# CFGpp-diffusion/CFGpp

Measured on NVIDIA H100. Metric: images/sec (device-timed) SDXL 1024x1024 NFE=50 ddim_cfg++, higher is better.
Workload: dtype f16

## Files before the change

cfgpp_b200/csrc/attention.cu:

```cuda
#include <cmath>

#include "attention.cuh"
#include "common.cuh"

namespace cfgpp {

void attn_configure();

namespace {

constexpr int BQ = 64;
constexpr int BKV = 64;
constexpr int kThreads = 128;
constexpr int ATOM_BYTES = 64 * 64 * 2;

template <int HD>
struct ACfg {
  static constexpr int NA = HD / 64;
  static constexpr int TILE_BYTES = NA * ATOM_BYTES;
  static constexpr int SMEM_BYTES = TILE_BYTES * 5 + 1024 + 64;
  static_assert(SMEM_BYTES <= 232448, "shared memory overflow");
};

CFGPP_DEVICE uint32_t tile_off(int row, int chunk) {
  return (chunk >> 3) * ATOM_BYTES + row * 128 + (((chunk & 7) ^ (row & 7)) << 4);
}

template <int HD, bool IP>
CFGPP_DEVICE void attn_body(const AttnParams& p, const CUtensorMap* map_q, const CUtensorMap* map_k,
                            const CUtensorMap* map_v, const CUtensorMap* map_k2, const CUtensorMap* map_v2) {
  using A = ACfg<HD>;
  constexpr int NA = A::NA;
  constexpr int TILE_BYTES = A::TILE_BYTES;
  extern __shared__ uint8_t smem_raw[];
  const uint32_t raw_addr = smem_u32(smem_raw);
  uint8_t* smem = smem_raw + (((raw_addr + 1023u) & ~1023u) - raw_addr);
  uint8_t* sQ = smem;
  uint8_t* sK = sQ + TILE_BYTES;
  uint8_t* sV = sK + 2 * TILE_BYTES;
  uint64_t* bars = reinterpret_cast<uint64_t*>(sV + 2 * TILE_BYTES);
  uint64_t* q_full = bars;
  uint64_t* kv_full = bars + 1;

  const int warp = threadIdx.x >> 5;
  const int lane = threadIdx.x & 31;
  const int q0 = blockIdx.x * BQ;
  const int head = blockIdx.y;
  const int batch = blockIdx.z;
  const int n_tiles = (p.Nkv + BKV - 1) / BKV;

  if (threadIdx.x == 0) {
    tma_prefetch_desc(map_q);
    tma_prefetch_desc(map_k);
    tma_prefetch_desc(map_v);
    mbar_init(q_full, 1);
    mbar_init(&kv_full[0], 1);
    mbar_init(&kv_full[1], 1);
    fence_barrier_init();
  }
  __syncthreads();
  pdl_launch_dependents();
  pdl_wait();
  const float ip_scale = IP ? *p.ip_scale : 0.f;
  const bool ip = IP && ip_scale != 0.f;
  const int n_fills = n_tiles + (ip ? 1 : 0);

  auto load_kv = [&](int j) {
    const int s = j & 1;
    const bool image = IP && j == n_tiles;
    const CUtensorMap* mk = image ? map_k2 : map_k;
    const CUtensorMap* mv = image ? map_v2 : map_v;
    const int row = image ? 0 : j * BKV;
    mbar_arrive_expect_tx(&kv_full[s], 2 * TILE_BYTES);
#pragma unroll
    for (int a = 0; a < NA; ++a) {
      tma_load_3d(sK + s * TILE_BYTES + a * ATOM_BYTES, mk, &kv_full[s], head * HD + a * 64, row, batch);
      tma_load_3d(sV + s * TILE_BYTES + a * ATOM_BYTES, mv, &kv_full[s], head * HD + a * 64, row, batch);
    }
  };
  if (threadIdx.x == 0) {
    if (IP) {
      tma_prefetch_desc(map_k2);
      tma_prefetch_desc(map_v2);
    }
    mbar_arrive_expect_tx(q_full, TILE_BYTES);
#pragma unroll
    for (int a = 0; a < NA; ++a) tma_load_3d(sQ + a * ATOM_BYTES, map_q, q_full, head * HD + a * 64, q0, batch);
    load_kv(0);
    if (n_fills > 1) load_kv(1);
  }

  const float c = p.scale_log2e;
  float o[HD / 8][4];
#pragma unroll
  for (int n = 0; n < HD / 8; ++n) o[n][0] = o[n][1] = o[n][2] = o[n][3] = 0.f;
  float m_run[2] = {-INFINITY, -INFINITY}, l_run[2] = {0.f, 0.f};
  const uint32_t q_base = smem_u32(sQ);
  const int qrow_ld = warp * 16 + (lane & 15);
  auto scores = [&](uint32_t k_base, int valid, float (&sc)[BKV / 8][4]) {
#pragma unroll
    for (int n = 0; n < BKV / 8; ++n) sc[n][0] = sc[n][1] = sc[n][2] = sc[n][3] = 0.f;
#pragma unroll
    for (int kk = 0; kk < HD / 16; ++kk) {
      uint32_t a[4];
      ldmatrix_x4(q_base + tile_off(qrow_ld, 2 * kk + (lane >> 4)), a[0], a[1], a[2], a[3]);
#pragma unroll
      for (int n2 = 0; n2 < BKV / 16; ++n2) {
        const int krow = n2 * 16 + (lane & 7) + ((lane >> 4) << 3);
        uint32_t b0, b1, b2, b3;
        ldmatrix_x4(k_base + tile_off(krow, 2 * kk + ((lane >> 3) & 1)), b0, b1, b2, b3);
        mma_16816(sc[2 * n2], a, b0, b1);
        mma_16816(sc[2 * n2 + 1], a, b2, b3);
      }
    }
    if (valid < BKV) {
#pragma unroll
      for (int n = 0; n < BKV / 8; ++n) {
        const int col = n * 8 + 2 * (lane & 3);
        if (col >= valid) sc[n][0] = sc[n][2] = -INFINITY;
        if (col + 1 >= valid) sc[n][1] = sc[n][3] = -INFINITY;
      }
    }
  };
  mbar_wait(q_full, 0);

  for (int j = 0; j < n_tiles; ++j) {
    const int s = j & 1;
    mbar_wait(&kv_full[s], (j >> 1) & 1);
    const uint32_t k_base = smem_u32(sK + s * TILE_BYTES);
    const uint32_t v_base = smem_u32(sV + s * TILE_BYTES);
    float sc[BKV / 8][4];
    scores(k_base, p.Nkv - j * BKV, sc);
    float alpha[2];
#pragma unroll
    for (int h = 0; h < 2; ++h) {
      float mx = -INFINITY;
#pragma unroll
      for (int n = 0; n < BKV / 8; ++n) mx = fmaxf(mx, fmaxf(sc[n][2 * h], sc[n][2 * h + 1]));
      mx = fmaxf(mx, __shfl_xor_sync(0xffffffffu, mx, 1));
      mx = fmaxf(mx, __shfl_xor_sync(0xffffffffu, mx, 2));
      const float m_new = fmaxf(m_run[h], mx);
      alpha[h] = fast_exp2((m_run[h] - m_new) * c);
      m_run[h] = m_new;
    }
    float rs[2] = {0.f, 0.f};
    uint32_t pa[BKV / 8][2];
#pragma unroll
    for (int n = 0; n < BKV / 8; ++n) {
#pragma unroll
      for (int h = 0; h < 2; ++h) {
        const float mc = m_run[h] * c;
        const float p0 = fast_exp2(sc[n][2 * h] * c - mc);
        const float p1 = fast_exp2(sc[n][2 * h + 1] * c - mc);
        rs[h] += p0 + p1;
        pa[n][h] = pack_half2(p0, p1);
      }
    }
#pragma unroll
    for (int h = 0; h < 2; ++h) l_run[h] = l_run[h] * alpha[h] + rs[h];
#pragma unroll
    for (int n = 0; n < HD / 8; ++n) {
      o[n][0] *= alpha[0];
      o[n][1] *= alpha[0];
      o[n][2] *= alpha[1];
      o[n][3] *= alpha[1];
    }
#pragma unroll
    for (int t = 0; t < BKV / 16; ++t) {
      const uint32_t a[4] = {pa[2 * t][0], pa[2 * t][1], pa[2 * t + 1][0], pa[2 * t + 1][1]};
      const int vrow = t * 16 + (lane & 7) + (((lane >> 3) & 1) << 3);
#pragma unroll
      for (int d2 = 0; d2 < HD / 16; ++d2) {
        uint32_t b0, b1, b2, b3;
        ldmatrix_x4_trans(v_base + tile_off(vrow, 2 * d2 + (lane >> 4)), b0, b1, b2, b3);
        mma_16816(o[2 * d2], a, b0, b1);
        mma_16816(o[2 * d2 + 1], a, b2, b3);
      }
    }
    __syncthreads();
    if (threadIdx.x == 0 && j + 2 < n_fills) load_kv(j + 2);
  }

  float inv_l[2];
#pragma unroll
  for (int h = 0; h < 2; ++h) {
    float l = l_run[h];
    l += __shfl_xor_sync(0xffffffffu, l, 1);
    l += __shfl_xor_sync(0xffffffffu, l, 2);
    inv_l[h] = 1.0f / l;
  }
  if (ip) {
    const int s = n_tiles & 1;
    mbar_wait(&kv_full[s], (n_tiles >> 1) & 1);
    const uint32_t v_base = smem_u32(sV + s * TILE_BYTES);
    float sc[BKV / 8][4];
    scores(smem_u32(sK + s * TILE_BYTES), p.Nkv2, sc);
    float mc[2], inv_l2[2];
#pragma unroll
    for (int h = 0; h < 2; ++h) {
      float mx = -INFINITY;
#pragma unroll
      for (int n = 0; n < BKV / 8; ++n) mx = fmaxf(mx, fmaxf(sc[n][2 * h], sc[n][2 * h + 1]));
      mx = fmaxf(mx, __shfl_xor_sync(0xffffffffu, mx, 1));
      mx = fmaxf(mx, __shfl_xor_sync(0xffffffffu, mx, 2));
      mc[h] = mx * c;
    }
    float rs[2] = {0.f, 0.f};
    uint32_t pa[BKV / 8][2];
#pragma unroll
    for (int n = 0; n < BKV / 8; ++n) {
#pragma unroll
      for (int h = 0; h < 2; ++h) {
        const float p0 = fast_exp2(sc[n][2 * h] * c - mc[h]);
        const float p1 = fast_exp2(sc[n][2 * h + 1] * c - mc[h]);
        rs[h] += p0 + p1;
        pa[n][h] = pack_half2(p0, p1);
      }
    }
#pragma unroll
    for (int h = 0; h < 2; ++h) {
      float l = rs[h];
      l += __shfl_xor_sync(0xffffffffu, l, 1);
      l += __shfl_xor_sync(0xffffffffu, l, 2);
      inv_l2[h] = 1.0f / l;
    }
    const int k_steps = (p.Nkv2 + 15) / 16;
#pragma unroll
    for (int d2 = 0; d2 < HD / 16; ++d2) {
      float acc[2][4] = {{0.f, 0.f, 0.f, 0.f}, {0.f, 0.f, 0.f, 0.f}};
#pragma unroll
      for (int t = 0; t < BKV / 16; ++t) {
        if (t >= k_steps) break;
        const uint32_t a[4] = {pa[2 * t][0], pa[2 * t][1], pa[2 * t + 1][0], pa[2 * t + 1][1]};
        const int vrow = t * 16 + (lane & 7) + (((lane >> 3) & 1) << 3);
        uint32_t b0, b1, b2, b3;
        ldmatrix_x4_trans(v_base + tile_off(vrow, 2 * d2 + (lane >> 4)), b0, b1, b2, b3);
        mma_16816(acc[0], a, b0, b1);
        mma_16816(acc[1], a, b2, b3);
      }
#pragma unroll
      for (int i = 0; i < 2; ++i)
#pragma unroll
        for (int e = 0; e < 4; ++e)
          o[2 * d2 + i][e] = o[2 * d2 + i][e] * inv_l[e >> 1] + ip_scale * (acc[i][e] * inv_l2[e >> 1]);
    }
    inv_l[0] = inv_l[1] = 1.0f;
  }
#pragma unroll
  for (int h = 0; h < 2; ++h) {
    const int qrow = q0 + warp * 16 + (lane >> 2) + 8 * h;
    if (qrow >= p.Nq) continue;
    __half* dst = p.out + (static_cast<size_t>(batch) * p.Nq + qrow) * p.ldo + head * HD + 2 * (lane & 3);
#pragma unroll
    for (int n = 0; n < HD / 8; ++n)
      *reinterpret_cast<uint32_t*>(dst + n * 8) = pack_half2(o[n][2 * h] * inv_l[h], o[n][2 * h + 1] * inv_l[h]);
  }
}

template <int HD>
__global__ void __launch_bounds__(kThreads)
attn_kernel(const AttnParams p, const __grid_constant__ CUtensorMap map_q, const __grid_constant__ CUtensorMap map_k,
            const __grid_constant__ CUtensorMap map_v) {
  attn_body<HD, false>(p, &map_q, &map_k, &map_v, nullptr, nullptr);
}

template <int HD>
__global__ void __launch_bounds__(kThreads)
attn_ip_kernel(const AttnParams p, const __grid_constant__ CUtensorMap map_q, const __grid_constant__ CUtensorMap map_k,
               const __grid_constant__ CUtensorMap map_v, const __grid_constant__ CUtensorMap map_k2,
               const __grid_constant__ CUtensorMap map_v2) {
  attn_body<HD, true>(p, &map_q, &map_k, &map_v, &map_k2, &map_v2);
}

CUtensorMap make_head_map(const __half* base, int ld, int B, int N, int cols) {
  uint64_t dims[3] = {(uint64_t)cols, (uint64_t)N, (uint64_t)B};
  uint64_t strides[2] = {(uint64_t)ld * 2, (uint64_t)N * ld * 2};
  uint32_t box[3] = {64, 64, 1};
  return make_tmap_f16(base, 3, dims, strides, box);
}

template <int HD>
void configure_one() {
  CFGPP_CHECK_CUDA(cudaFuncSetAttribute(attn_kernel<HD>, cudaFuncAttributeMaxDynamicSharedMemorySize,
                                        ACfg<HD>::SMEM_BYTES));
  CFGPP_CHECK_CUDA(cudaFuncSetAttribute(attn_ip_kernel<HD>, cudaFuncAttributeMaxDynamicSharedMemorySize,
                                        ACfg<HD>::SMEM_BYTES));
}

template <int HD>
void launch(const AttnOp& op, cudaStream_t stream) {
  dim3 grid((op.p.Nq + BQ - 1) / BQ, op.p.H, op.p.B);
  if (op.p.ip_scale)
    launch_pdl(attn_ip_kernel<HD>, grid, dim3(kThreads), ACfg<HD>::SMEM_BYTES, stream, op.p, op.map_q, op.map_k,
               op.map_v, op.map_k2, op.map_v2);
  else
    launch_pdl(attn_kernel<HD>, grid, dim3(kThreads), ACfg<HD>::SMEM_BYTES, stream, op.p, op.map_q, op.map_k,
               op.map_v);
}

}

int attn_padded_head_dim(int head_dim) { return ((head_dim + 63) / 64) * 64; }

AttnOp make_attn_op(const __half* q, int ldq, const __half* k, int ldk, const __half* v, int ldv, __half* out,
                    int ldo, int B, int H, int Nq, int Nkv, int head_dim) {
  AttnOp op{};
  CFGPP_REQUIRE(Nkv >= 1 && Nq >= 1, "empty attention");
  CFGPP_REQUIRE(ldo % 8 == 0, "ldo must be a multiple of 8");
  CFGPP_REQUIRE(head_dim >= 8 && head_dim <= 192, "attention supports head_dim <= 192");
  const int hdp = attn_padded_head_dim(head_dim);
  op.hd_pad = hdp;
  op.head_dim = head_dim;
  op.p.B = B; op.p.H = H; op.p.Nq = Nq; op.p.Nkv = Nkv; op.p.ldo = ldo; op.p.out = out;
  op.p.scale_log2e = (1.0f / sqrtf(static_cast<float>(head_dim))) * 1.4426950408889634f;
  op.map_q = make_head_map(q, ldq, B, Nq, H * hdp);
  op.map_k = make_head_map(k, ldk, B, Nkv, H * hdp);
  op.map_v = make_head_map(v, ldv, B, Nkv, H * hdp);
  return op;
}

AttnOp make_attn_ip_op(const __half* q, int ldq, const __half* k, int ldk, const __half* v, int ldv, const __half* k2,
                       int ldk2, const __half* v2, int ldv2, int Nkv2, const float* ip_scale, __half* out, int ldo,
                       int B, int H, int Nq, int Nkv, int head_dim) {
  CFGPP_REQUIRE(Nkv2 >= 1 && Nkv2 <= 64, "the image segment holds 1..64 tokens");
  CFGPP_REQUIRE(ip_scale != nullptr, "the image segment needs its scale word");
  AttnOp op = make_attn_op(q, ldq, k, ldk, v, ldv, out, ldo, B, H, Nq, Nkv, head_dim);
  op.p.Nkv2 = Nkv2;
  op.p.ip_scale = ip_scale;
  op.map_k2 = make_head_map(k2, ldk2, B, Nkv2, H * op.hd_pad);
  op.map_v2 = make_head_map(v2, ldv2, B, Nkv2, H * op.hd_pad);
  return op;
}

void attn_configure() {
  static bool done = false;
  if (done) return;
  configure_one<64>();
  configure_one<128>();
  configure_one<192>();
  done = true;
}

void run_attn_op(const AttnOp& op, cudaStream_t stream) {
  attn_configure();
  switch (op.hd_pad) {
    case 64: return launch<64>(op, stream);
    case 128: return launch<128>(op, stream);
    case 192: return launch<192>(op, stream);
    default: throw Error(-1, "unsupported padded head dim");
  }
}

}
```

cfgpp_b200/csrc/common.cuh:

```cuda
#pragma once
#include <cuda.h>
#include <cuda_fp16.h>
#include <cuda_runtime.h>
#include <stdint.h>
#include <stdio.h>

namespace cfgpp {

#define CFGPP_DEVICE __device__ __forceinline__

CFGPP_DEVICE uint32_t smem_u32(const void* p) {
  return static_cast<uint32_t>(__cvta_generic_to_shared(p));
}

CFGPP_DEVICE void pdl_launch_dependents() { asm volatile("griddepcontrol.launch_dependents;" ::: "memory"); }
CFGPP_DEVICE void pdl_wait() { asm volatile("griddepcontrol.wait;" ::: "memory"); }

CFGPP_DEVICE void mbar_init(uint64_t* bar, uint32_t count) {
  asm volatile("mbarrier.init.shared::cta.b64 [%0], %1;" ::"r"(smem_u32(bar)), "r"(count));
}
CFGPP_DEVICE void fence_barrier_init() {
  asm volatile("fence.mbarrier_init.release.cluster;" ::: "memory");
}
CFGPP_DEVICE void mbar_arrive_expect_tx(uint64_t* bar, uint32_t bytes) {
  asm volatile("mbarrier.arrive.expect_tx.shared::cta.b64 _, [%0], %1;" ::"r"(smem_u32(bar)), "r"(bytes)
               : "memory");
}
CFGPP_DEVICE void mbar_arrive(uint64_t* bar) {
  asm volatile("mbarrier.arrive.shared::cta.b64 _, [%0];" ::"r"(smem_u32(bar)) : "memory");
}
CFGPP_DEVICE uint32_t mbar_try_wait(uint64_t* bar, uint32_t parity) {
  uint32_t ok;
  asm volatile(
      "{\n\t"
      ".reg .pred P1;\n\t"
      "mbarrier.try_wait.parity.shared::cta.b64 P1, [%1], %2;\n\t"
      "selp.u32 %0, 1, 0, P1;\n\t"
      "}"
      : "=r"(ok)
      : "r"(smem_u32(bar)), "r"(parity)
      : "memory");
  return ok;
}
#ifndef CFGPP_MBAR_SLEEP_NS
#define CFGPP_MBAR_SLEEP_NS 1000000
#endif
CFGPP_DEVICE uint32_t mbar_try_wait_sleep(uint64_t* bar, uint32_t parity) {
  uint32_t ok;
  asm volatile(
      "{\n\t"
      ".reg .pred P1;\n\t"
      "mbarrier.try_wait.parity.shared::cta.b64 P1, [%1], %2, %3;\n\t"
      "selp.u32 %0, 1, 0, P1;\n\t"
      "}"
      : "=r"(ok)
      : "r"(smem_u32(bar)), "r"(parity), "r"(CFGPP_MBAR_SLEEP_NS)
      : "memory");
  return ok;
}
CFGPP_DEVICE void mbar_wait(uint64_t* bar, uint32_t parity) {
  if (mbar_try_wait(bar, parity)) return;
  const long long t0 = clock64();
#if CFGPP_MBAR_SLEEP_NS > 0
  while (!mbar_try_wait_sleep(bar, parity)) {
#else
  while (!mbar_try_wait(bar, parity)) {
#endif
    if (clock64() - t0 > 4000000000LL) {
      printf("cfgpp: mbarrier wait timeout (block %d thread %d bar 0x%x parity %u)\n", blockIdx.x, threadIdx.x,
             smem_u32(bar), parity);
      __trap();
    }
  }
}

CFGPP_DEVICE void mbar_wait_nocall(uint64_t* bar, uint32_t parity) {
  if (mbar_try_wait(bar, parity)) return;
  const long long t0 = clock64();
  while (!mbar_try_wait(bar, parity)) {
    if (clock64() - t0 > 4000000000LL) __trap();
  }
}

CFGPP_DEVICE void tma_prefetch_desc(const CUtensorMap* map) {
  asm volatile("prefetch.tensormap [%0];" ::"l"(reinterpret_cast<uint64_t>(map)) : "memory");
}
CFGPP_DEVICE void tma_load_2d(void* smem_dst, const CUtensorMap* map, uint64_t* bar, int c0, int c1) {
  asm volatile(
      "cp.async.bulk.tensor.2d.shared::cluster.global.mbarrier::complete_tx::bytes [%0], [%1, {%3, %4}], [%2];"
      ::"r"(smem_u32(smem_dst)), "l"(reinterpret_cast<uint64_t>(map)), "r"(smem_u32(bar)), "r"(c0), "r"(c1)
      : "memory");
}
CFGPP_DEVICE void tma_load_3d(void* smem_dst, const CUtensorMap* map, uint64_t* bar, int c0, int c1, int c2) {
  asm volatile(
      "cp.async.bulk.tensor.3d.shared::cluster.global.mbarrier::complete_tx::bytes [%0], [%1, {%3, %4, %5}], [%2];"
      ::"r"(smem_u32(smem_dst)), "l"(reinterpret_cast<uint64_t>(map)), "r"(smem_u32(bar)), "r"(c0), "r"(c1),
      "r"(c2)
      : "memory");
}
CFGPP_DEVICE void tma_load_4d(void* smem_dst, const CUtensorMap* map, uint64_t* bar, int c0, int c1, int c2,
                              int c3) {
  asm volatile(
      "cp.async.bulk.tensor.4d.shared::cluster.global.mbarrier::complete_tx::bytes [%0], [%1, {%3, %4, %5, %6}], "
      "[%2];" ::"r"(smem_u32(smem_dst)),
      "l"(reinterpret_cast<uint64_t>(map)), "r"(smem_u32(bar)), "r"(c0), "r"(c1), "r"(c2), "r"(c3)
      : "memory");
}
CFGPP_DEVICE void tma_load_im2col_4d(void* smem_dst, const CUtensorMap* map, uint64_t* bar, int c, int w, int h, int n,
                                     uint16_t off_w, uint16_t off_h) {
  asm volatile(
      "cp.async.bulk.tensor.4d.shared::cluster.global.im2col.mbarrier::complete_tx::bytes [%0], [%1, {%3, %4, %5, %6}], "
      "[%2], {%7, %8};" ::"r"(smem_u32(smem_dst)),
      "l"(reinterpret_cast<uint64_t>(map)), "r"(smem_u32(bar)), "r"(c), "r"(w), "r"(h), "r"(n), "h"(off_w), "h"(off_h)
      : "memory");
}

CFGPP_DEVICE void tma_store_2d(const CUtensorMap* map, const void* smem_src, int c0, int c1) {
  asm volatile("cp.async.bulk.tensor.2d.global.shared::cta.bulk_group [%0, {%2, %3}], [%1];" ::"l"(
                   reinterpret_cast<uint64_t>(map)),
               "r"(smem_u32(smem_src)), "r"(c0), "r"(c1)
               : "memory");
}
CFGPP_DEVICE void tma_store_commit() { asm volatile("cp.async.bulk.commit_group;" ::: "memory"); }
CFGPP_DEVICE void tma_store_wait_read0() { asm volatile("cp.async.bulk.wait_group.read 0;" ::: "memory"); }
CFGPP_DEVICE void tma_store_wait0() { asm volatile("cp.async.bulk.wait_group 0;" ::: "memory"); }
CFGPP_DEVICE void named_bar_sync(int id, int nthreads) {
  asm volatile("bar.sync %0, %1;" ::"r"(id), "r"(nthreads) : "memory");
}

CFGPP_DEVICE void fence_proxy_async_smem() { asm volatile("fence.proxy.async.shared::cta;" ::: "memory"); }

template <uint32_t N>
CFGPP_DEVICE void setmaxnreg_inc() { asm volatile("setmaxnreg.inc.sync.aligned.u32 %0;" ::"n"(N)); }
template <uint32_t N>
CFGPP_DEVICE void setmaxnreg_dec() { asm volatile("setmaxnreg.dec.sync.aligned.u32 %0;" ::"n"(N)); }

CFGPP_DEVICE void wgmma_fence() { asm volatile("wgmma.fence.sync.aligned;" ::: "memory"); }
CFGPP_DEVICE void wgmma_commit() { asm volatile("wgmma.commit_group.sync.aligned;" ::: "memory"); }
template <int N>
CFGPP_DEVICE void wgmma_wait() { asm volatile("wgmma.wait_group.sync.aligned %0;" ::"n"(N) : "memory"); }
template <int N>
CFGPP_DEVICE void fence_acc(float (&d)[N]) {
#pragma unroll
  for (int i = 0; i < N; ++i) asm volatile("" : "+f"(d[i])::"memory");
}

CFGPP_DEVICE uint64_t make_wgmma_desc_sw128(uint32_t smem_addr) {
  uint64_t d = 0;
  d |= static_cast<uint64_t>((smem_addr >> 4) & 0x3FFF);
  d |= static_cast<uint64_t>(1) << 16;
  d |= static_cast<uint64_t>(1024 >> 4) << 32;
  d |= static_cast<uint64_t>(1) << 62;
  return d;
}

#define CFGPP_D8(i) "+f"(d[i]), "+f"(d[i + 1]), "+f"(d[i + 2]), "+f"(d[i + 3]), "+f"(d[i + 4]), "+f"(d[i + 5]), \
                    "+f"(d[i + 6]), "+f"(d[i + 7])
template <int N>
CFGPP_DEVICE void wgmma_f16(float (&d)[N / 2], uint64_t a_desc, uint64_t b_desc, uint32_t scale_d);
template <>
CFGPP_DEVICE void wgmma_f16<64>(float (&d)[32], uint64_t a_desc, uint64_t b_desc, uint32_t scale_d) {
  asm volatile("{\n.reg .pred p;\nsetp.ne.b32 p, %34, 0;\nwgmma.mma_async.sync.aligned.m64n64k16.f32.f16.f16 {"
               "%0,%1,%2,%3,%4,%5,%6,%7,%8,%9,%10,%11,%12,%13,%14,%15,%16,%17,%18,%19,%20,%21,%22,%23,%24,%25,%26,"
               "%27,%28,%29,%30,%31"
               "}, %32, %33, p, 1, 1, 0, 0;\n}\n"
               : CFGPP_D8(0), CFGPP_D8(8), CFGPP_D8(16), CFGPP_D8(24)
               : "l"(a_desc), "l"(b_desc), "r"(scale_d)
               : "memory");
}
template <>
CFGPP_DEVICE void wgmma_f16<128>(float (&d)[64], uint64_t a_desc, uint64_t b_desc, uint32_t scale_d) {
  asm volatile("{\n.reg .pred p;\nsetp.ne.b32 p, %66, 0;\nwgmma.mma_async.sync.aligned.m64n128k16.f32.f16.f16 {"
               "%0,%1,%2,%3,%4,%5,%6,%7,%8,%9,%10,%11,%12,%13,%14,%15,%16,%17,%18,%19,%20,%21,%22,%23,%24,%25,%26,"
               "%27,%28,%29,%30,%31,%32,%33,%34,%35,%36,%37,%38,%39,%40,%41,%42,%43,%44,%45,%46,%47,%48,%49,%50,%51,"
               "%52,%53,%54,%55,%56,%57,%58,%59,%60,%61,%62,%63"
               "}, %64, %65, p, 1, 1, 0, 0;\n}\n"
               : CFGPP_D8(0), CFGPP_D8(8), CFGPP_D8(16), CFGPP_D8(24), CFGPP_D8(32), CFGPP_D8(40), CFGPP_D8(48), CFGPP_D8(56)
               : "l"(a_desc), "l"(b_desc), "r"(scale_d)
               : "memory");
}
template <>
CFGPP_DEVICE void wgmma_f16<160>(float (&d)[80], uint64_t a_desc, uint64_t b_desc, uint32_t scale_d) {
  asm volatile("{\n.reg .pred p;\nsetp.ne.b32 p, %82, 0;\nwgmma.mma_async.sync.aligned.m64n160k16.f32.f16.f16 {"
               "%0,%1,%2,%3,%4,%5,%6,%7,%8,%9,%10,%11,%12,%13,%14,%15,%16,%17,%18,%19,%20,%21,%22,%23,%24,%25,%26,"
               "%27,%28,%29,%30,%31,%32,%33,%34,%35,%36,%37,%38,%39,%40,%41,%42,%43,%44,%45,%46,%47,%48,%49,%50,%51,"
               "%52,%53,%54,%55,%56,%57,%58,%59,%60,%61,%62,%63,%64,%65,%66,%67,%68,%69,%70,%71,%72,%73,%74,%75,%76,"
               "%77,%78,%79"
               "}, %80, %81, p, 1, 1, 0, 0;\n}\n"
               : CFGPP_D8(0), CFGPP_D8(8), CFGPP_D8(16), CFGPP_D8(24), CFGPP_D8(32), CFGPP_D8(40), CFGPP_D8(48), CFGPP_D8(56), CFGPP_D8(64), CFGPP_D8(72)
               : "l"(a_desc), "l"(b_desc), "r"(scale_d)
               : "memory");
}
template <>
CFGPP_DEVICE void wgmma_f16<256>(float (&d)[128], uint64_t a_desc, uint64_t b_desc, uint32_t scale_d) {
  asm volatile("{\n.reg .pred p;\nsetp.ne.b32 p, %130, 0;\nwgmma.mma_async.sync.aligned.m64n256k16.f32.f16.f16 {"
               "%0,%1,%2,%3,%4,%5,%6,%7,%8,%9,%10,%11,%12,%13,%14,%15,%16,%17,%18,%19,%20,%21,%22,%23,%24,%25,%26,"
               "%27,%28,%29,%30,%31,%32,%33,%34,%35,%36,%37,%38,%39,%40,%41,%42,%43,%44,%45,%46,%47,%48,%49,%50,%51,"
               "%52,%53,%54,%55,%56,%57,%58,%59,%60,%61,%62,%63,%64,%65,%66,%67,%68,%69,%70,%71,%72,%73,%74,%75,%76,"
               "%77,%78,%79,%80,%81,%82,%83,%84,%85,%86,%87,%88,%89,%90,%91,%92,%93,%94,%95,%96,%97,%98,%99,%100,"
               "%101,%102,%103,%104,%105,%106,%107,%108,%109,%110,%111,%112,%113,%114,%115,%116,%117,%118,%119,%120,"
               "%121,%122,%123,%124,%125,%126,%127"
               "}, %128, %129, p, 1, 1, 0, 0;\n}\n"
               : CFGPP_D8(0), CFGPP_D8(8), CFGPP_D8(16), CFGPP_D8(24), CFGPP_D8(32), CFGPP_D8(40), CFGPP_D8(48), CFGPP_D8(56), CFGPP_D8(64), CFGPP_D8(72), CFGPP_D8(80), CFGPP_D8(88), CFGPP_D8(96), CFGPP_D8(104), CFGPP_D8(112), CFGPP_D8(120)
               : "l"(a_desc), "l"(b_desc), "r"(scale_d)
               : "memory");
}
#undef CFGPP_D8

CFGPP_DEVICE void ldmatrix_x4(uint32_t addr, uint32_t& r0, uint32_t& r1, uint32_t& r2, uint32_t& r3) {
  asm volatile("ldmatrix.sync.aligned.m8n8.x4.shared.b16 {%0, %1, %2, %3}, [%4];"
               : "=r"(r0), "=r"(r1), "=r"(r2), "=r"(r3)
               : "r"(addr));
}
CFGPP_DEVICE void ldmatrix_x4_trans(uint32_t addr, uint32_t& r0, uint32_t& r1, uint32_t& r2, uint32_t& r3) {
  asm volatile("ldmatrix.sync.aligned.m8n8.x4.trans.shared.b16 {%0, %1, %2, %3}, [%4];"
               : "=r"(r0), "=r"(r1), "=r"(r2), "=r"(r3)
               : "r"(addr));
}
CFGPP_DEVICE void mma_16816(float (&d)[4], const uint32_t (&a)[4], uint32_t b0, uint32_t b1) {
  asm volatile(
      "mma.sync.aligned.m16n8k16.row.col.f32.f16.f16.f32 {%0, %1, %2, %3}, {%4, %5, %6, %7}, {%8, %9}, "
      "{%0, %1, %2, %3};"
      : "+f"(d[0]), "+f"(d[1]), "+f"(d[2]), "+f"(d[3])
      : "r"(a[0]), "r"(a[1]), "r"(a[2]), "r"(a[3]), "r"(b0), "r"(b1));
}

CFGPP_DEVICE unsigned long long globaltimer_ns() {
  unsigned long long t;
  asm volatile("mov.u64 %0, %%globaltimer;" : "=l"(t));
  return t;
}

CFGPP_DEVICE float silu_f(float x) { return __fdividef(x, 1.0f + __expf(-x)); }
CFGPP_DEVICE float gelu_erf_f(float x) { return 0.5f * x * (1.0f + erff(x * 0.70710678118654752440f)); }
CFGPP_DEVICE float gelu_erf_fast_f(float x) {
  const float az = fabsf(x) * 0.70710678118654752440f;
  const float t = __fdividef(1.0f, fmaf(0.3275911f, az, 1.0f));
  float e;
  asm("ex2.approx.ftz.f32 %0, %1;" : "=f"(e) : "f"(-az * az * 1.4426950408889634f));
  float p = 1.061405429f;
  p = fmaf(p, t, -1.453152027f);
  p = fmaf(p, t, 1.421413741f);
  p = fmaf(p, t, -0.284496736f);
  p = fmaf(p, t, 0.254829592f);
  const float q = p * t * e;
  return 0.5f * x * (x >= 0.f ? 2.0f - q : q);
}

CFGPP_DEVICE float fast_exp2(float x) {
  float y;
  asm("ex2.approx.ftz.f32 %0, %1;" : "=f"(y) : "f"(x));
  return y;
}

CFGPP_DEVICE uint32_t pack_half2(float a, float b) {
  __half2 h = __floats2half2_rn(a, b);
  return *reinterpret_cast<uint32_t*>(&h);
}

}
```

Baseline: 0.5933.

## Add warp-specialized wgmma attention kernel for head dim 64

Replaces the generic head-dim-64 attention path with a dedicated kernel. A producer warp issues TMA loads of 128-row K/V tiles into a 4-stage mbarrier ring, while two consumer warpgroups run wgmma for QK^T and register-sourced PV. The consumers alternate turns through named barriers so one group's softmax overlaps the other's tensor-core work, and registers are rebalanced with setmaxnreg. It uses larger 128x128 tiles at one CTA per SM, which costs occupancy and adds more complex synchronization.

```diff
diff --git a/cfgpp_b200/csrc/attention.cu b/cfgpp_b200/csrc/attention.cu
--- a/cfgpp_b200/csrc/attention.cu
+++ b/cfgpp_b200/csrc/attention.cu
@@ -1,4 +1,5 @@
 #include <cmath>
+#include <type_traits>
 
 #include "attention.cuh"
 #include "common.cuh"
@@ -272,6 +273,265 @@
   attn_body<HD, true>(p, &map_q, &map_k, &map_v, &map_k2, &map_v2);
 }
 
+constexpr int W_BQ = 128;
+constexpr int W_BKV = 128;
+constexpr int W_STAGES = 4;
+constexpr int W_THREADS = 384;
+constexpr int W_KV_BYTES = 2 * ATOM_BYTES;
+constexpr int W_SMEM_BYTES = 2 * ATOM_BYTES + W_STAGES * 2 * W_KV_BYTES + 1024 + 256;
+static_assert(W_SMEM_BYTES <= 232448, "shared memory overflow");
+constexpr int kTurnBar = 1;
+
+template <bool IP>
+CFGPP_DEVICE void attn64_body(const AttnParams& p, const CUtensorMap* map_q, const CUtensorMap* map_k,
+                              const CUtensorMap* map_v, const CUtensorMap* map_k2, const CUtensorMap* map_v2) {
+  extern __shared__ uint8_t smem_raw[];
+  const uint32_t raw_addr = smem_u32(smem_raw);
+  uint8_t* smem = smem_raw + (((raw_addr + 1023u) & ~1023u) - raw_addr);
+  uint8_t* sQ = smem;
+  uint8_t* sK = sQ + 2 * ATOM_BYTES;
+  uint8_t* sV = sK + W_STAGES * W_KV_BYTES;
+  uint64_t* q_full = reinterpret_cast<uint64_t*>(sV + W_STAGES * W_KV_BYTES);
+  uint64_t* full = q_full + 1;
+  uint64_t* empty = full + W_STAGES;
+
+  const int warp = threadIdx.x >> 5;
+  const int lane = threadIdx.x & 31;
+  const int q0 = blockIdx.x * W_BQ;
+  const int head = blockIdx.y;
+  const int batch = blockIdx.z;
+  const int n_tiles = (p.Nkv + W_BKV - 1) / W_BKV;
+
+  if (threadIdx.x == 0) {
+    mbar_init(q_full, 1);
+    for (int s = 0; s < W_STAGES; ++s) {
+      mbar_init(&full[s], 1);
+      mbar_init(&empty[s], 8);
+    }
+    fence_barrier_init();
+  }
+  __syncthreads();
+  pdl_launch_dependents();
+  pdl_wait();
+  const float ip_scale = IP ? *p.ip_scale : 0.f;
+  const bool ip = IP && ip_scale != 0.f;
+
+  if (warp >= 8) {
+    setmaxnreg_dec<40>();
+    if (threadIdx.x == 256) {
+      tma_prefetch_desc(map_q);
+      tma_prefetch_desc(map_k);
+      tma_prefetch_desc(map_v);
+      if (IP) {
+        tma_prefetch_desc(map_k2);
+        tma_prefetch_desc(map_v2);
+      }
+      mbar_arrive_expect_tx(q_full, 2 * ATOM_BYTES);
+      tma_load_3d(sQ, map_q, q_full, head * 64, q0, batch);
+      tma_load_3d(sQ + ATOM_BYTES, map_q, q_full, head * 64, q0 + 64, batch);
+      for (int f = 0; f < n_tiles + (IP ? 1 : 0); ++f) {
+        const int s = f % W_STAGES;
+        mbar_wait_nocall(&empty[s], ((f / W_STAGES) & 1) ^ 1);
+        uint8_t* k_dst = sK + s * W_KV_BYTES;
+        uint8_t* v_dst = sV + s * W_KV_BYTES;
+        if (IP && f == n_tiles) {
+          mbar_arrive_expect_tx(&full[s], 2 * ATOM_BYTES);
+          tma_load_3d(k_dst, map_k2, &full[s], head * 64, 0, batch);
+          tma_load_3d(v_dst, map_v2, &full[s], head * 64, 0, batch);
+        } else {
+          mbar_arrive_expect_tx(&full[s], 4 * ATOM_BYTES);
+          for (int h = 0; h < 2; ++h) {
+            tma_load_3d(k_dst + h * ATOM_BYTES, map_k, &full[s], head * 64, f * W_BKV + h * 64, batch);
+            tma_load_3d(v_dst + h * ATOM_BYTES, map_v, &full[s], head * 64, f * W_BKV + h * 64, batch);
+          }
+        }
+      }
+    }
+    return;
+  }
+
+  setmaxnreg_inc<232>();
+  const int wg = warp >> 2;
+  const float c = p.scale_log2e;
+  float sc[W_BKV / 2];
+  float o[32];
+#pragma unroll
+  for (int i = 0; i < 32; ++i) o[i] = 0.f;
+  uint32_t pa[W_BKV / 4];
+  float m_run[2] = {-INFINITY, -INFINITY}, l_run[2] = {0.f, 0.f};
+  const uint64_t q_desc = make_wgmma_desc_sw128(smem_u32(sQ + wg * ATOM_BYTES));
+
+  auto issue_s = [&](int s) {
+    const uint64_t k_desc = make_wgmma_desc_sw128(smem_u32(sK + s * W_KV_BYTES));
+#pragma unroll
+    for (int k = 0; k < 4; ++k) wgmma_f16<W_BKV>(sc, q_desc + 2 * k, k_desc + 2 * k, k != 0 ? 1u : 0u);
+  };
+  auto issue_pv = [&](float (&acc)[32], int s, auto rows) {
+    const uint64_t v_desc = make_wgmma_desc_sw128_mn(smem_u32(sV + s * W_KV_BYTES));
+#pragma unroll
+    for (int t = 0; t < decltype(rows)::value / 16; ++t) {
+      const uint32_t a[4] = {pa[4 * t], pa[4 * t + 1], pa[4 * t + 2], pa[4 * t + 3]};
+      wgmma_f16_rs_tb64(acc, a, v_desc + 128 * t, 1u);
+    }
+  };
+  auto softmax = [&](int valid, float (&m)[2], float (&l)[2], float (&acc)[32]) {
+    if (valid < W_BKV) {
+#pragma unroll
+      for (int n = 0; n < W_BKV / 8; ++n) {
+        const int col = n * 8 + 2 * (lane & 3);
+        if (col >= valid) sc[4 * n] = sc[4 * n + 2] = -INFINITY;
+        if (col + 1 >= valid) sc[4 * n + 1] = sc[4 * n + 3] = -INFINITY;
+      }
+    }
+    float alpha[2];
+#pragma unroll
+    for (int h = 0; h < 2; ++h) {
+      float mx = -INFINITY;
+#pragma unroll
+      for (int n = 0; n < W_BKV / 8; ++n) mx = fmaxf(mx, fmaxf(sc[4 * n + 2 * h], sc[4 * n + 2 * h + 1]));
+      mx = fmaxf(mx, __shfl_xor_sync(0xffffffffu, mx, 1));
+      mx = fmaxf(mx, __shfl_xor_sync(0xffffffffu, mx, 2));
+      const float m_new = fmaxf(m[h], mx);
+      alpha[h] = fast_exp2((m[h] - m_new) * c);
+      m[h] = m_new;
+    }
+    float rs[2] = {0.f, 0.f};
+#pragma unroll
+    for (int n = 0; n < W_BKV / 8; ++n) {
+#pragma unroll
+      for (int h = 0; h < 2; ++h) {
+        const float mc = m[h] * c;
+        const float p0 = fast_exp2(sc[4 * n + 2 * h] * c - mc);
+        const float p1 = fast_exp2(sc[4 * n + 2 * h + 1] * c - mc);
+        rs[h] += p0 + p1;
+        pa[2 * n + h] = pack_half2(p0, p1);
+      }
+    }
+#pragma unroll
+    for (int h = 0; h < 2; ++h) l[h] = l[h] * alpha[h] + rs[h];
+#pragma unroll
+    for (int n = 0; n < 8; ++n) {
+      acc[4 * n] *= alpha[0];
+      acc[4 * n + 1] *= alpha[0];
+      acc[4 * n + 2] *= alpha[1];
+      acc[4 * n + 3] *= alpha[1];
+    }
+  };
+
+  mbar_wait_nocall(q_full, 0);
+  if (wg == 1) named_bar_arrive(kTurnBar, 256);
+  constexpr std::integral_constant<int, W_BKV> kAllRows{};
+  mbar_wait_nocall(&full[0], 0);
+  named_bar_sync(kTurnBar + wg, 256);
+  wgmma_fence();
+  issue_s(0);
+  wgmma_commit();
+  named_bar_arrive(kTurnBar + (wg ^ 1), 256);
+  wgmma_wait<0>();
+  fence_acc(sc);
+  softmax(p.Nkv, m_run, l_run, o);
+  for (int j = 1; j < n_tiles; ++j) {
+    const int s = j % W_STAGES;
+    const int sp = (j - 1) % W_STAGES;
+    mbar_wait_nocall(&full[s], (j / W_STAGES) & 1);
+    named_bar_sync(kTurnBar + wg, 256);
+    wgmma_fence();
+    issue_s(s);
+    issue_pv(o, sp, kAllRows);
+    wgmma_commit();
+    named_bar_arrive(kTurnBar + (wg ^ 1), 256);
+    wgmma_wait<0>();
+    fence_acc(sc);
+    fence_acc(o);
+    fence_acc(pa);
+    if (lane == 0) mbar_arrive(&empty[sp]);
+    softmax(p.Nkv - j * W_BKV, m_run, l_run, o);
+  }
+  const int s_last = (n_tiles - 1) % W_STAGES;
+  named_bar_sync(kTurnBar + wg, 256);
+  wgmma_fence();
+  issue_pv(o, s_last, kAllRows);
+  wgmma_commit();
+  if (wg == 0) named_bar_arrive(kTurnBar + 1, 256);
+  wgmma_wait<0>();
+  fence_acc(o);
+  fence_acc(pa);
+  if (lane == 0) mbar_arrive(&empty[s_last]);
+
+  float inv_l[2];
+#pragma unroll
+  for (int h = 0; h < 2; ++h) {
+    float l = l_run[h];
+    l += __shfl_xor_sync(0xffffffffu, l, 1);
+    l += __shfl_xor_sync(0xffffffffu, l, 2);
+    inv_l[h] = 1.0f / l;
+  }
+  if constexpr (IP) {
+    const int s = n_tiles % W_STAGES;
+    mbar_wait_nocall(&full[s], (n_tiles / W_STAGES) & 1);
+    wgmma_fence();
+    issue_s(s);
+    wgmma_commit();
+    wgmma_wait<0>();
+    fence_acc(sc);
+    float m2[2] = {-INFINITY, -INFINITY}, l2[2] = {0.f, 0.f};
+    float o2[32];
+#pragma unroll
+    for (int i = 0; i < 32; ++i) o2[i] = 0.f;
+    softmax(p.Nkv2, m2, l2, o2);
+    wgmma_fence();
+    issue_pv(o2, s, std::integral_constant<int, 64>{});
+    wgmma_commit();
+    wgmma_wait<0>();
+    fence_acc(o2);
+    fence_acc(pa);
+#pragma unroll
+    for (int h = 0; h < 2; ++h) {
+      float l = l2[h];
+      l += __shfl_xor_sync(0xffffffffu, l, 1);
+      l += __shfl_xor_sync(0xffffffffu, l, 2);
+      l2[h] = 1.0f / l;
+    }
+#pragma unroll
+    for (int i = 0; i < 32; ++i) {
+      const float fold = o[i] * inv_l[(i >> 1) & 1] + ip_scale * (o2[i] * l2[(i >> 1) & 1]);
+      o[i] = ip ? fold : o[i];
+    }
+    if (ip) inv_l[0] = inv_l[1] = 1.0f;
+  }
+#pragma unroll
+  for (int h = 0; h < 2; ++h) {
+    const int qrow = q0 + warp * 16 + (lane >> 2) + 8 * h;
+    if (qrow >= p.Nq) continue;
+    __half* dst = p.out + (static_cast<size_t>(batch) * p.Nq + qrow) * p.ldo + head * 64 + 2 * (lane & 3);
+#pragma unroll
+    for (int n = 0; n < 8; ++n)
+      *reinterpret_cast<uint32_t*>(dst + n * 8) = pack_half2(o[4 * n + 2 * h] * inv_l[h], o[4 * n + 2 * h + 1] * inv_l[h]);
+  }
+}
+
+__global__ void __launch_bounds__(W_THREADS, 1)
+attn64_kernel(const AttnParams p, const __grid_constant__ CUtensorMap map_q, const __grid_constant__ CUtensorMap map_k,
+              const __grid_constant__ CUtensorMap map_v) {
+  attn64_body<false>(p, &map_q, &map_k, &map_v, nullptr, nullptr);
+}
+
+__global__ void __launch_bounds__(W_THREADS, 1)
+attn64_ip_kernel(const AttnParams p, const __grid_constant__ CUtensorMap map_q,
+                 const __grid_constant__ CUtensorMap map_k, const __grid_constant__ CUtensorMap map_v,
+                 const __grid_constant__ CUtensorMap map_k2, const __grid_constant__ CUtensorMap map_v2) {
+  attn64_body<true>(p, &map_q, &map_k, &map_v, &map_k2, &map_v2);
+}
+
+void launch64(const AttnOp& op, cudaStream_t stream) {
+  dim3 grid((op.p.Nq + W_BQ - 1) / W_BQ, op.p.H, op.p.B);
+  if (op.p.ip_scale)
+    launch_pdl(attn64_ip_kernel, grid, dim3(W_THREADS), W_SMEM_BYTES, stream, op.p, op.map_q, op.map_k, op.map_v,
+               op.map_k2, op.map_v2);
+  else
+    launch_pdl(attn64_kernel, grid, dim3(W_THREADS), W_SMEM_BYTES, stream, op.p, op.map_q, op.map_k, op.map_v);
+}
+
 CUtensorMap make_head_map(const __half* base, int ld, int B, int N, int cols) {
   uint64_t dims[3] = {(uint64_t)cols, (uint64_t)N, (uint64_t)B};
   uint64_t strides[2] = {(uint64_t)ld * 2, (uint64_t)N * ld * 2};
@@ -335,7 +595,8 @@
 void attn_configure() {
   static bool done = false;
   if (done) return;
-  configure_one<64>();
+  CFGPP_CHECK_CUDA(cudaFuncSetAttribute(attn64_kernel, cudaFuncAttributeMaxDynamicSharedMemorySize, W_SMEM_BYTES));
+  CFGPP_CHECK_CUDA(cudaFuncSetAttribute(attn64_ip_kernel, cudaFuncAttributeMaxDynamicSharedMemorySize, W_SMEM_BYTES));
   configure_one<128>();
   configure_one<192>();
   done = true;
@@ -344,7 +605,7 @@
 void run_attn_op(const AttnOp& op, cudaStream_t stream) {
   attn_configure();
   switch (op.hd_pad) {
-    case 64: return launch<64>(op, stream);
+    case 64: return launch64(op, stream);
     case 128: return launch<128>(op, stream);
     case 192: return launch<192>(op, stream);
     default: throw Error(-1, "unsupported padded head dim");
diff --git a/cfgpp_b200/csrc/common.cuh b/cfgpp_b200/csrc/common.cuh
--- a/cfgpp_b200/csrc/common.cuh
+++ b/cfgpp_b200/csrc/common.cuh
@@ -127,6 +127,9 @@
 CFGPP_DEVICE void named_bar_sync(int id, int nthreads) {
   asm volatile("bar.sync %0, %1;" ::"r"(id), "r"(nthreads) : "memory");
 }
+CFGPP_DEVICE void named_bar_arrive(int id, int nthreads) {
+  asm volatile("bar.arrive %0, %1;" ::"r"(id), "r"(nthreads) : "memory");
+}
 
 CFGPP_DEVICE void fence_proxy_async_smem() { asm volatile("fence.proxy.async.shared::cta;" ::: "memory"); }
 
@@ -143,6 +146,11 @@
 CFGPP_DEVICE void fence_acc(float (&d)[N]) {
 #pragma unroll
   for (int i = 0; i < N; ++i) asm volatile("" : "+f"(d[i])::"memory");
+}
+template <int N>
+CFGPP_DEVICE void fence_acc(uint32_t (&a)[N]) {
+#pragma unroll
+  for (int i = 0; i < N; ++i) asm volatile("" : "+r"(a[i])::"memory");
 }
 
 CFGPP_DEVICE uint64_t make_wgmma_desc_sw128(uint32_t smem_addr) {
@@ -203,6 +211,25 @@
                "}, %128, %129, p, 1, 1, 0, 0;\n}\n"
                : CFGPP_D8(0), CFGPP_D8(8), CFGPP_D8(16), CFGPP_D8(24), CFGPP_D8(32), CFGPP_D8(40), CFGPP_D8(48), CFGPP_D8(56), CFGPP_D8(64), CFGPP_D8(72), CFGPP_D8(80), CFGPP_D8(88), CFGPP_D8(96), CFGPP_D8(104), CFGPP_D8(112), CFGPP_D8(120)
                : "l"(a_desc), "l"(b_desc), "r"(scale_d)
+               : "memory");
+}
+
+CFGPP_DEVICE uint64_t make_wgmma_desc_sw128_mn(uint32_t smem_addr) {
+  uint64_t d = 0;
+  d |= static_cast<uint64_t>((smem_addr >> 4) & 0x3FFF);
+  d |= static_cast<uint64_t>(1024 >> 4) << 16;
+  d |= static_cast<uint64_t>(1024 >> 4) << 32;
+  d |= static_cast<uint64_t>(1) << 62;
+  return d;
+}
+
+CFGPP_DEVICE void wgmma_f16_rs_tb64(float (&d)[32], const uint32_t (&a)[4], uint64_t b_desc, uint32_t scale_d) {
+  asm volatile("{\n.reg .pred p;\nsetp.ne.b32 p, %37, 0;\nwgmma.mma_async.sync.aligned.m64n64k16.f32.f16.f16 {"
+               "%0,%1,%2,%3,%4,%5,%6,%7,%8,%9,%10,%11,%12,%13,%14,%15,%16,%17,%18,%19,%20,%21,%22,%23,%24,%25,%26,"
+               "%27,%28,%29,%30,%31"
+               "}, {%32,%33,%34,%35}, %36, p, 1, 1, 1;\n}\n"
+               : CFGPP_D8(0), CFGPP_D8(8), CFGPP_D8(16), CFGPP_D8(24)
+               : "r"(a[0]), "r"(a[1]), "r"(a[2]), "r"(a[3]), "l"(b_desc), "r"(scale_d)
                : "memory");
 }
 #undef CFGPP_D8
```

Measured after the change: 0.6221, median of 6. 4.8% higher.
